# ambicuity/Distributed-LLM-Training-and-Inference-System

Hardware: AMD Instinct MI355X
Metric: tokens/sec (node) GPT-7B train (higher is better)
Workload: dtype bf16; 1 GPU; model=gpt-7b, global_batch=16, seq_len=2048, parallelism=dp1, micro_batch=16, grad_accum=1, activation_checkpoint=none, layout=planner

## Files before the change

llmctl/config/knobs.py:

```python

from __future__ import annotations

import contextlib
import dataclasses
import os
from dataclasses import dataclass, fields
from typing import Any, Dict, Iterator, Optional

ENV = "LLMCTL_KNOBS"


@dataclass(frozen=True)
class PerfKnobs:
    gemm64: bool = True
    gemm64_config: int = 304
    fwd64: str = "auto"
    dgrad64: str = "fused"
    wgrad_kernel: bool = True
    swiglu_bwd: str = "side"
    dgrad_transpose: bool = True
    wt_side_stream: bool = True
    fused_fwd: bool = False
    rope_inplace: bool = True
    fused_rope_attn: bool = True
    moe_pad: bool = True
    overlap_optimizer: bool = False
    gemm_tuning: bool = True
    fa_split: int = -1
    fa_prio: int = 1
    fa_nw: int = 4
    dkv: int = 2
    dkv_nwg: int = 0
    async_tp: bool = True
    async_tp_save_full: bool = False
    cp_zigzag: bool = True
    decode_fused: bool = True
    decode_splits: int = 0
    decode_v3: int = 1
    skinny_gemm: str = "auto"
    prefill_swiglu: bool = True
    prefill_fa: bool = True
    prefill_norm_fold: bool = True
    mixed_steps: bool = True
    custom_ar: bool = True
    tp_graphs: bool = True
    async_decode: bool = True
    tp_fused_decode: bool = True
    moe_decode_fused: bool = True

    def as_dict(self) -> Dict[str, Any]:
        return dataclasses.asdict(self)


NATIVE = ("fa_split", "fa_prio", "fa_nw", "dkv", "dkv_nwg", "decode_splits", "decode_v3")
_FIELDS = {f.name: f for f in fields(PerfKnobs)}


def _coerce(name: str, value: Any) -> Any:
    if name not in _FIELDS:
        raise KeyError(f"unknown performance knob {name!r} (known: {', '.join(sorted(_FIELDS))})")
    typ = _FIELDS[name].type
    if typ in ("bool", bool):
        if isinstance(value, str):
            v = value.strip().lower()
            if v not in ("1", "0", "true", "false", "on", "off", "yes", "no"):
                raise ValueError(f"knob {name}: expected a boolean, got {value!r}")
            return v in ("1", "true", "on", "yes")
        return bool(value)
    if typ in ("int", int):
        return int(value)
    return str(value)


def parse_env(spec: Optional[str]) -> Dict[str, Any]:
    out: Dict[str, Any] = {}
    for part in (spec or "").split(","):
        part = part.strip()
        if not part:
            continue
        if "=" not in part:
            raise ValueError(f"{ENV}: expected name=value, got {part!r}")
        k, v = part.split("=", 1)
        out[k.strip()] = _coerce(k.strip(), v.strip())
    return out


_RETIRED_ENV = ("LLMCTL_SIDE_DGRAD", "LLMCTL_DECODE_ATTN_QKV", "LLMCTL_GEMM64_CONFIG", "LLMCTL_SKINNY")
_warned: set = set()


def _warn_retired_env() -> None:
    import warnings

    names = [f"LLMCTL_{n.upper()}" for n in _FIELDS] + list(_RETIRED_ENV)
    for n in names:
        if n in os.environ and n not in _warned:
            _warned.add(n)
            warnings.warn(f"{n} is no longer read (performance switches are knobs now): set "
                          f"{ENV}=\"{n[7:].lower()}=<value>\" or the [perf] config table instead", stacklevel=3)


def resolve(overrides: Optional[Dict[str, Any]] = None, env: bool = True) -> PerfKnobs:
    _warn_retired_env()
    kw = {k: _coerce(k, v) for k, v in (overrides or {}).items()}
    if env:
        kw.update(parse_env(os.environ.get(ENV)))
    return PerfKnobs(**kw)


_ACTIVE: PerfKnobs = resolve()


def knobs() -> PerfKnobs:
    return _ACTIVE


def push_native(k: Optional[PerfKnobs] = None) -> bool:
    k = k or _ACTIVE
    try:
        from llmctl.ops import _lib

        if not _lib.loaded():
            return False
        import torch

        for name in NATIVE:
            torch.ops.llmctl.set_knob(name, int(getattr(k, name)))
        return True
    except Exception:
        return False


def apply(k: PerfKnobs) -> PerfKnobs:
    global _ACTIVE
    _ACTIVE = k
    push_native(k)
    return k


def use(k: PerfKnobs) -> PerfKnobs:
    if k is not _ACTIVE:
        apply(k)
    return k


def with_env(k: PerfKnobs) -> PerfKnobs:
    env = parse_env(os.environ.get(ENV))
    return dataclasses.replace(k, **env) if env else k


def configure(overrides: Optional[Dict[str, Any]] = None) -> PerfKnobs:
    return apply(resolve(overrides))


@contextlib.contextmanager
def override(**kw: Any) -> Iterator[PerfKnobs]:
    old = _ACTIVE
    new = dataclasses.replace(old, **{k: _coerce(k, v) for k, v in kw.items()})
    apply(new)
    try:
        yield new
    finally:
        apply(old)
```

llmctl/ops/csrc/flash_attn_fwd.hip:

```cpp
#include <cstdlib>

#include "attn_common.h"

namespace llmctl {
using namespace attn;
namespace {

constexpr int KB = 64;
constexpr float kRescaleTh = 8.f;

struct FwdArgs {
  const unsigned short* q;
  const unsigned short* k;
  const unsigned short* v;
  unsigned short* o;
  float* lse;
  int B, S, Hq, Hkv;
  long q_sb, q_ss, q_sh;
  long k_sb, k_ss, k_sh;
  long v_sb, v_ss, v_sh;
  long o_sb, o_ss, o_sh;
  float scale_log2;
  const int* doc;
  unsigned short* o_part;
  float* lse_part;
  int prio;
};

template <int HD, bool CAUSAL, bool DOC = false, bool SPLIT = false, int NW = 4, int NBUF = 2>
__global__ __launch_bounds__(NW * 64, 2) void fa_fwd_kernel(FwdArgs a) {
  constexpr int QB = NW * 32;
  constexpr int NTHR = NW * 64;
  constexpr int NKS = HD / 16;
  constexpr int NDB = HD / 32;
  constexpr int ROWB = HD * 2;
  constexpr int TILE = KB * ROWB;
  constexpr int PPW = TILE / 1024 / NW;
  constexpr int SLOT = 2 * TILE;
  static_assert(PPW * NW * 1024 == TILE, "pieces must split evenly over the waves");
  __shared__ __attribute__((aligned(1024))) unsigned char smem[NBUF * SLOT];

  const int tid = threadIdx.x;
  const int lane = tid & 63;
  const int wave = __builtin_amdgcn_readfirstlane(tid >> 6);
  const int r = lane & 31, hh = lane >> 5;
  const int nqb = (a.S + QB - 1) / QB;
  const int BH = a.B * a.Hq;
  int bh, rest;
  if (SPLIT || BH % 8) {
    bh = blockIdx.x % BH;
    rest = blockIdx.x / BH;
  } else {
    const int x = blockIdx.x & 7, j = blockIdx.x >> 3;
    bh = x * (BH >> 3) + j / nqb;
    rest = j % nqb;
  }
  const int part = SPLIT ? rest & 1 : 0;
  const int qblk = nqb - 1 - (SPLIT ? rest >> 1 : rest);
  const int b = bh / a.Hq, hq = bh % a.Hq;
  const int hk = hq / (a.Hq / a.Hkv);
  const int q_row0 = qblk * QB + wave * 32;
  const int my_q = q_row0 + r;

  const unsigned short* Qp = a.q + b * a.q_sb + hq * a.q_sh;
  const unsigned short* Kp = a.k + b * a.k_sb + hk * a.k_sh;
  const unsigned short* Vp = a.v + b * a.v_sb + hk * a.v_sh;

#pragma unroll
  for (int i = 0; i < NBUF * SLOT / (NTHR * 16); ++i)
    *reinterpret_cast<uint4*>(smem + i * NTHR * 16 + tid * 16) = make_uint4(0, 0, 0, 0);

  bf16x8_t qf[NKS];
#pragma unroll
  for (int ks = 0; ks < NKS; ++ks) {
    uint4 u = make_uint4(0, 0, 0, 0);
    if (my_q < a.S) u = gload16(Qp + (long)my_q * a.q_ss + ks * 16 + 8 * hh);
    qf[ks] = __builtin_bit_cast(bf16x8_t, u);
  }

  f32x16 o[NDB];
#pragma unroll
  for (int d = 0; d < NDB; ++d)
#pragma unroll
    for (int i = 0; i < 16; ++i) o[d][i] = 0.f;
  float m_i = -INFINITY, l_i = 0.f;

  const int kv_end = CAUSAL ? min(a.S, qblk * QB + QB) : a.S;
  int ntiles = (kv_end + KB - 1) / KB;
  int my_start = 0, w_min = 0, w_max = 0, t0 = 0;
  if constexpr (DOC) {
    const int* ds = a.doc + (long)b * a.S;
    my_start = ds[min(my_q, a.S - 1)];
    w_min = __builtin_amdgcn_readfirstlane(ds[min(q_row0, a.S - 1)]);
    w_max = __builtin_amdgcn_readfirstlane(ds[min(q_row0 + 31, a.S - 1)]);
    t0 = __builtin_amdgcn_readfirstlane(ds[min(qblk * QB, a.S - 1)]) / KB;
  }
  if constexpr (SPLIT) {
    const int mid = (t0 + ntiles) / 2;
    if (part == 0) ntiles = mid;
    else t0 = mid;
  }

  unsigned vk[PPW], vv[PPW];
#pragma unroll
  for (int i = 0; i < PPW; ++i) {
    const int byte = (i * NW + wave) * 1024 + lane * 16;
    const int row = byte / ROWB, pch = (byte % ROWB) >> 4;
    vk[i] = (unsigned)((row * a.k_ss + ((pch ^ swz_row<HD>(row)) << 3)) * 2);
    vv[i] = (unsigned)((row * a.v_ss + ((pch ^ swz_tr<HD>(row)) << 3)) * 2);
  }
  const unsigned lds0 = lds_addr(smem);
  int ik0 = t0 * KB;
  const unsigned short* kc = Kp + (long)ik0 * a.k_ss;
  const unsigned short* vc = Vp + (long)ik0 * a.v_ss;
  const long k_step = (long)KB * a.k_ss, v_step = (long)KB * a.v_ss;
  auto issue = [&](auto slot_c) __attribute__((always_inline)) {
    constexpr int SLC = decltype(slot_c)::value;
    const int nk = min(KB, a.S - ik0);
    i32x4_t rk = buf_rsrc(kc, (unsigned)(((nk - 1) * a.k_ss + HD) * 2));
    i32x4_t rv = buf_rsrc(vc, (unsigned)(((nk - 1) * a.v_ss + HD) * 2));
    asm volatile("s_nop 4" : "+s"(rk), "+s"(rv));
    const unsigned slot = lds0 + (unsigned)(SLC * SLOT) + wave * 1024;
#pragma unroll
    for (int i = 0; i < PPW; ++i) {
      buf_dma16(rk, vk[i], slot + i * NW * 1024);
      buf_dma16(rv, vv[i], slot + TILE + i * NW * 1024);
    }
    ik0 += KB;
    kc += k_step;
    vc += v_step;
  };

  const float c = a.scale_log2;
  const int key_hi = CAUSAL ? min(my_q, a.S - 1) : a.S - 1;
  int vlo[NDB], vhi[NDB];
#pragma unroll
  for (int d = 0; d < NDB; ++d) tr_frag_offs<HD>(d * 32, lane, vlo[d], vhi[d]);
  int kofs[NKS];
#pragma unroll
  for (int ks = 0; ks < NKS; ++ks) kofs[ks] = row_off<HD>(r, 2 * ks + hh);
#pragma unroll
  for (int ks = 0; ks < NKS; ++ks) asm volatile("" ::"v"(qf[ks]));
  auto tile = [&](bool need_mask, const unsigned char* Ks, const unsigned char* Vs, int kv0) __attribute__((always_inline)) {
    if (a.prio) __builtin_amdgcn_s_setprio(1);
    f32x16 s[2];
#pragma unroll
    for (int kb = 0; kb < 2; ++kb) {
#pragma unroll
      for (int i = 0; i < 16; ++i) s[kb][i] = 0.f;
#pragma unroll
      for (int ks = 0; ks < NKS; ++ks) s[kb] = mfma32(lds_read_b128(Ks, kb * 32 * (HD * 2) + kofs[ks]), qf[ks], s[kb]);
    }
    if (need_mask) {
#pragma unroll
      for (int kb = 0; kb < 2; ++kb)
#pragma unroll
        for (int i = 0; i < 16; ++i) {
          const int key = kv0 + kb * 32 + acc_row(i, hh);
          bool ok = key <= key_hi;
          if constexpr (DOC) ok = ok && key >= my_start;
          s[kb][i] = ok ? s[kb][i] : -INFINITY;
        }
    }
    if (a.prio) __builtin_amdgcn_s_setprio(0);
    float mx = s[0][0];
#pragma unroll
    for (int kb = 0; kb < 2; ++kb)
#pragma unroll
      for (int i = (kb == 0 ? 1 : 0); i < 16; ++i) mx = fmaxf(mx, s[kb][i]);
    mx = xor32_max(mx) * c;
    const bool grow = __builtin_amdgcn_ballot_w64(mx > m_i + kRescaleTh) != 0;
    const float m_new = grow ? fmaxf(m_i, mx) : m_i;
    const float nm = (m_new == -INFINITY) ? 0.f : -m_new;
    float rs = 0.f;
    bf16x8_t pb[2][2];
#pragma unroll
    for (int kb = 0; kb < 2; ++kb) {
      float p[16];
#pragma unroll
      for (int i = 0; i < 16; ++i) {
        p[i] = fast_exp2(__builtin_fmaf(s[kb][i], c, nm));
        rs += p[i];
      }
      pb[kb][0] = to_bf16x8(p);
      pb[kb][1] = to_bf16x8(p + 8);
    }
    rs = xor32_add(rs);
    if (grow) {
      const float alpha = fast_exp2(m_i + nm);
      l_i *= alpha;
#pragma unroll
      for (int d = 0; d < NDB; ++d)
#pragma unroll
        for (int i = 0; i < 16; ++i) o[d][i] *= alpha;
    }
    l_i += rs;
    m_i = m_new;
    if (a.prio) __builtin_amdgcn_s_setprio(1);
#pragma unroll
    for (int kb = 0; kb < 2; ++kb)
#pragma unroll
      for (int st = 0; st < 2; ++st)
#pragma unroll
        for (int d = 0; d < NDB; ++d) o[d] = mfma32(tr_frag_at<HD>(Vs, kb * 32 + 16 * st, vlo[d], vhi[d]), pb[kb][st], o[d]);
    if (a.prio) __builtin_amdgcn_s_setprio(0);
  };

  __syncthreads();
  auto step = [&](auto slot_c, int t) __attribute__((always_inline)) {
    constexpr int SL = decltype(slot_c)::value;
    if constexpr (NBUF == 3) {
      if (t + 1 < ntiles) vm_wait_n<2 * PPW>();
      else vm_wait_n<0>();
    } else {
      vm_wait_n<0>();
    }
    __builtin_amdgcn_s_barrier();
    if (t + NBUF - 1 < ntiles) issue(std::integral_constant<int, (SL + NBUF - 1) % NBUF>{});
    const int kv0 = t * KB;
    bool live = true;
    if constexpr (CAUSAL) live = kv0 <= q_row0 + 31;
    if constexpr (DOC) live = live && kv0 + KB > w_min;
    if (live) {
      const bool need_mask = (CAUSAL && kv0 + KB - 1 > q_row0) || (kv0 + KB > a.S) || (DOC && kv0 < w_max);
      tile(need_mask, smem + SL * SLOT, smem + SL * SLOT + TILE, kv0);
    }
  };
  if (t0 < ntiles) issue(std::integral_constant<int, 0>{});
  if constexpr (NBUF == 3)
    if (t0 + 1 < ntiles) issue(std::integral_constant<int, 1>{});
  for (int t = t0; t < ntiles; t += NBUF) {
    step(std::integral_constant<int, 0>{}, t);
    if (t + 1 < ntiles) step(std::integral_constant<int, 1>{}, t + 1);
    if constexpr (NBUF == 3)
      if (t + 2 < ntiles) step(std::integral_constant<int, 2>{}, t + 2);
  }

  if constexpr (SPLIT) {
    if (my_q < a.S) {
      const float inv = l_i > 0.f ? 1.f / l_i : 0.f;
      unsigned short* Op = a.o_part + ((((long)part * a.B + b) * a.S + my_q) * a.Hq + hq) * HD;
#pragma unroll
      for (int d = 0; d < NDB; ++d)
#pragma unroll
        for (int g = 0; g < 4; ++g) {
          const int col = d * 32 + 8 * g + 4 * hh;
          unsigned short w4[4];
#pragma unroll
          for (int j = 0; j < 4; ++j) w4[j] = f2bf(o[d][4 * g + j] * inv);
          *reinterpret_cast<uint2*>(Op + col) =
              make_uint2((unsigned)w4[0] | ((unsigned)w4[1] << 16), (unsigned)w4[2] | ((unsigned)w4[3] << 16));
        }
      if (hh == 0)
        a.lse_part[(((long)part * a.B + b) * a.Hq + hq) * a.S + my_q] =
            (l_i > 0.f) ? (m_i + __log2f(l_i)) * 0.69314718055994531f : -INFINITY;
    }
    return;
  }
  if (my_q < a.S) {
    const float inv = l_i > 0.f ? 1.f / l_i : 0.f;
    unsigned short* Op = a.o + b * a.o_sb + (long)my_q * a.o_ss + hq * a.o_sh;
#pragma unroll
    for (int d = 0; d < NDB; ++d)
#pragma unroll
      for (int g = 0; g < 4; ++g) {
        const int col = d * 32 + 8 * g + 4 * hh;
        unsigned short w4[4];
#pragma unroll
        for (int j = 0; j < 4; ++j) w4[j] = f2bf(o[d][4 * g + j] * inv);
        *reinterpret_cast<uint2*>(Op + col) =
            make_uint2((unsigned)w4[0] | ((unsigned)w4[1] << 16), (unsigned)w4[2] | ((unsigned)w4[3] << 16));
      }
    if (hh == 0) {
      const float lse = (l_i > 0.f) ? (m_i + __log2f(l_i)) * 0.69314718055994531f : -INFINITY;
      a.lse[((long)b * a.Hq + hq) * a.S + my_q] = lse;
    }
  }
}

template <int HD>
__global__ __launch_bounds__(256) void fa_combine_kernel(const unsigned short* __restrict__ o_part,
                                                         const float* __restrict__ lse_part,
                                                         unsigned short* __restrict__ o, float* __restrict__ lse,
                                                         int B, int S, int Hq, long o_sb, long o_ss, long o_sh) {
  constexpr int LPR = HD / 8;
  const long gid = (long)blockIdx.x * 256 + threadIdx.x;
  const long row = gid / LPR;
  const int sub = gid % LPR;
  if (row >= (long)B * S * Hq) return;
  const int hq = row % Hq;
  const long bs = row / Hq;
  const int sq = bs % S;
  const int b = bs / S;
  const long li = ((long)b * Hq + hq) * S + sq;
  const long plane = (long)B * Hq * S;
  const float l0 = lse_part[li], l1 = lse_part[plane + li];
  const float m = fmaxf(l0, l1);
  float w0 = 0.f, w1 = 0.f, l = -INFINITY;
  if (m != -INFINITY) {
    const float e0 = __expf(l0 - m), e1 = __expf(l1 - m);
    l = m + __logf(e0 + e1);
    w0 = e0 / (e0 + e1);
    w1 = e1 / (e0 + e1);
  }
  const long ob = row * HD + sub * 8;
  const long osz = (long)B * S * Hq * HD;
  float out[8], x0[8], x1[8];
  load8(o_part + ob, x0);
  load8(o_part + osz + ob, x1);
#pragma unroll
  for (int j = 0; j < 8; ++j) out[j] = w0 * x0[j] + w1 * x1[j];
  store8(o + b * o_sb + (long)sq * o_ss + (long)hq * o_sh + sub * 8, out);
  if (sub == 0) lse[li] = l;
}

template <int NW, int NBUF>
std::tuple<at::Tensor, at::Tensor> fwd_launch(const at::Tensor& q, at::Tensor& o, at::Tensor& lse, FwdArgs& a, int B,
                                              int S, int Hq, int D, bool causal,
                                              const c10::optional<at::Tensor>& doc_start) {
  constexpr int QB = NW * 32, WG_PER_CU = NW == 4 ? 2 : 1;
  const int nqb = (S + QB - 1) / QB;
  dim3 grid((unsigned)(B * Hq * nqb)), block(NW * 64);
  auto s = stream();
  bool split = causal && !(doc_start.has_value() && doc_start->defined()) && nqb >= 4 &&
               (long)B * Hq * nqb <= (long)WG_PER_CU * num_cus();
  if (const int64_t e = knob("fa_split", -1); e == 0) split = false;
  else if (e == 1) split = causal && !(doc_start.has_value() && doc_start->defined()) && nqb >= 2;
  if (split) {
    auto o_part = at::empty({2, B, S, Hq, D}, q.options());
    auto lse_part = at::empty({2, B, Hq, S}, q.options().dtype(at::kFloat));
    a.o_part = bf_mut(o_part);
    a.lse_part = lse_part.data_ptr<float>();
    dim3 g2((unsigned)(2 * B * Hq * nqb));
    const long threads = (long)B * S * Hq * (D / 8);
    if (D == 128) {
      hipLaunchKernelGGL((fa_fwd_kernel<128, true, false, true, NW, NBUF>), g2, block, 0, s, a);
      hipLaunchKernelGGL(fa_combine_kernel<128>, dim3((threads + 255) / 256), dim3(256), 0, s, a.o_part, a.lse_part,
                         bf_mut(o), lse.data_ptr<float>(), B, S, Hq, o.stride(0), o.stride(1), o.stride(2));
    } else {
      hipLaunchKernelGGL((fa_fwd_kernel<64, true, false, true, NW, NBUF>), g2, block, 0, s, a);
      hipLaunchKernelGGL(fa_combine_kernel<64>, dim3((threads + 255) / 256), dim3(256), 0, s, a.o_part, a.lse_part,
                         bf_mut(o), lse.data_ptr<float>(), B, S, Hq, o.stride(0), o.stride(1), o.stride(2));
    }
    return {o, lse};
  }
  if (doc_start.has_value() && doc_start->defined()) {
    const at::Tensor& ds = *doc_start;
    LLMCTL_CHECK(causal, "flash_attn_fwd: doc_start (packed sequences) needs causal attention");
    LLMCTL_CHECK(ds.is_cuda() && ds.scalar_type() == at::kInt && ds.is_contiguous() && ds.dim() == 2 &&
                     ds.size(0) == B && ds.size(1) == S,
                 "flash_attn_fwd: doc_start must be contiguous int32 [B,S]");
    a.doc = ds.data_ptr<int>();
    if (D == 128) hipLaunchKernelGGL((fa_fwd_kernel<128, true, true, false, NW, NBUF>), grid, block, 0, s, a);
    else hipLaunchKernelGGL((fa_fwd_kernel<64, true, true, false, NW, NBUF>), grid, block, 0, s, a);
    return {o, lse};
  }
  if (D == 128) {
    if (causal) hipLaunchKernelGGL((fa_fwd_kernel<128, true, false, false, NW, NBUF>), grid, block, 0, s, a);
    else hipLaunchKernelGGL((fa_fwd_kernel<128, false, false, false, NW, NBUF>), grid, block, 0, s, a);
  } else {
    if (causal) hipLaunchKernelGGL((fa_fwd_kernel<64, true, false, false, NW, NBUF>), grid, block, 0, s, a);
    else hipLaunchKernelGGL((fa_fwd_kernel<64, false, false, false, NW, NBUF>), grid, block, 0, s, a);
  }
  return {o, lse};
}

}

std::tuple<at::Tensor, at::Tensor> flash_attn_fwd(const at::Tensor& q, const at::Tensor& k, const at::Tensor& v,
                                                  double scale, bool causal,
                                                  const c10::optional<at::Tensor>& doc_start) {
  LLMCTL_CHECK(q.is_cuda() && k.is_cuda() && v.is_cuda(), "flash_attn_fwd: GPU tensors");
  LLMCTL_CHECK(q.scalar_type() == at::kBFloat16 && k.scalar_type() == at::kBFloat16 &&
                   v.scalar_type() == at::kBFloat16,
               "flash_attn_fwd: bf16");
  LLMCTL_CHECK(q.dim() == 4 && k.dim() == 4 && v.dim() == 4, "q/k/v must be [B,S,H,D]");
  const int B = q.size(0), S = q.size(1), Hq = q.size(2), D = q.size(3);
  const int Hkv = k.size(2);
  LLMCTL_CHECK(k.size(0) == B && k.size(1) == S && v.sizes() == k.sizes() && k.size(3) == D,
               "k/v shape must be [B,S,Hkv,D] matching q");
  LLMCTL_CHECK(Hq % Hkv == 0, "Hq must be a multiple of Hkv");
  LLMCTL_CHECK(D == 64 || D == 128, "head_dim must be 64 or 128, got ", D);
  LLMCTL_CHECK(q.stride(3) == 1 && k.stride(3) == 1 && v.stride(3) == 1, "head_dim must be contiguous");
  for (const at::Tensor* t : {&q, &k, &v})
    LLMCTL_CHECK(t->stride(0) % 8 == 0 && t->stride(1) % 8 == 0 && t->stride(2) % 8 == 0 &&
                     (reinterpret_cast<uintptr_t>(t->data_ptr()) & 15) == 0,
                 "q/k/v strides must be multiples of 8 elements and 16-B aligned");
  const c10::DeviceGuard g(q.device());
  auto o = at::empty({B, S, Hq, D}, q.options());
  auto lse = at::empty({B, Hq, S}, q.options().dtype(at::kFloat));
  if (B * S * Hq == 0) return {o, lse};
  FwdArgs a{bf_ptr(q), bf_ptr(k), bf_ptr(v), bf_mut(o), lse.data_ptr<float>(), B, S, Hq, Hkv,
            q.stride(0), q.stride(1), q.stride(2), k.stride(0), k.stride(1), k.stride(2),
            v.stride(0), v.stride(1), v.stride(2), o.stride(0), o.stride(1), o.stride(2),
            (float)(scale * 1.4426950408889634), nullptr, nullptr, nullptr, 0};
  a.prio = knob("fa_prio", 1) != 0 ? 1 : 0;
  if (knob("fa_nw", 4) == 8) return fwd_launch<8, 3>(q, o, lse, a, B, S, Hq, D, causal, doc_start);
  return fwd_launch<4, 2>(q, o, lse, a, B, S, Hq, D, causal, doc_start);
}

TORCH_LIBRARY_IMPL(llmctl, CUDA, m) { m.impl("flash_attn_fwd", &flash_attn_fwd); }

}
```

Before: 30910 tokens/s.

## Add paced two-head flash-attention forward kernel and MFMA/LDS-read schedule hints

Adds a new 512-thread forward attention kernel in which two 4-wave halves each handle one head. It uses a ring of LDS buffers and explicit barriers so that K/V DMA, softmax and the MFMA phases of consecutive tiles overlap in a paced pipeline. The kernel sits behind a new fa_paced knob that is off by default, and it includes optional timestamp instrumentation. Separately, sched_group_barrier hints that interleave LDS reads with MFMAs are inserted into the existing forward kernel, which changes instruction scheduling on the default path. The hints can help or hurt latency hiding, and the paced kernel gives up occupancy for tighter overlap.

```diff
diff --git a/llmctl/config/knobs.py b/llmctl/config/knobs.py
--- a/llmctl/config/knobs.py
+++ b/llmctl/config/knobs.py
@@ -29,6 +29,7 @@
     fa_split: int = -1
     fa_prio: int = 1
     fa_nw: int = 4
+    fa_paced: int = -1
     dkv: int = 2
     dkv_nwg: int = 0
     async_tp: bool = True
@@ -52,7 +53,7 @@
         return dataclasses.asdict(self)
 
 
-NATIVE = ("fa_split", "fa_prio", "fa_nw", "dkv", "dkv_nwg", "decode_splits", "decode_v3")
+NATIVE = ("fa_split", "fa_prio", "fa_nw", "fa_paced", "dkv", "dkv_nwg", "decode_splits", "decode_v3")
 _FIELDS = {f.name: f for f in fields(PerfKnobs)}
 
 
diff --git a/llmctl/ops/csrc/flash_attn_fwd.hip b/llmctl/ops/csrc/flash_attn_fwd.hip
--- a/llmctl/ops/csrc/flash_attn_fwd.hip
+++ b/llmctl/ops/csrc/flash_attn_fwd.hip
@@ -8,6 +8,8 @@
 
 constexpr int KB = 64;
 constexpr float kRescaleTh = 8.f;
+constexpr int kStampMax = 192;
+constexpr bool kPacedAuto = false;
 
 struct FwdArgs {
   const unsigned short* q;
@@ -27,6 +29,16 @@
   int prio;
 };
 
+template <int I, int N, int PF, int R>
+__device__ __forceinline__ void mfma_stream_sched() {
+  if constexpr (I == 0) __builtin_amdgcn_sched_group_barrier(0x100, R * PF, 0);
+  if constexpr (I < N) {
+    __builtin_amdgcn_sched_group_barrier(0x008, 1, 0);
+    if constexpr (I + PF < N) __builtin_amdgcn_sched_group_barrier(0x100, R, 0);
+    mfma_stream_sched<I + 1, N, PF, R>();
+  }
+}
+
 template <int HD, bool CAUSAL, bool DOC = false, bool SPLIT = false, int NW = 4, int NBUF = 2>
 __global__ __launch_bounds__(NW * 64, 2) void fa_fwd_kernel(FwdArgs a) {
   constexpr int QB = NW * 32;
@@ -151,6 +163,7 @@
 #pragma unroll
       for (int ks = 0; ks < NKS; ++ks) s[kb] = mfma32(lds_read_b128(Ks, kb * 32 * (HD * 2) + kofs[ks]), qf[ks], s[kb]);
     }
+    mfma_stream_sched<0, 2 * NKS, 4, 1>();
     if (need_mask) {
 #pragma unroll
       for (int kb = 0; kb < 2; ++kb)
@@ -203,6 +216,7 @@
       for (int st = 0; st < 2; ++st)
 #pragma unroll
         for (int d = 0; d < NDB; ++d) o[d] = mfma32(tr_frag_at<HD>(Vs, kb * 32 + 16 * st, vlo[d], vhi[d]), pb[kb][st], o[d]);
+    mfma_stream_sched<0, 4 * NDB, 4, 2>();
     if (a.prio) __builtin_amdgcn_s_setprio(0);
   };
 
@@ -257,6 +271,283 @@
     }
     return;
   }
+  if (my_q < a.S) {
+    const float inv = l_i > 0.f ? 1.f / l_i : 0.f;
+    unsigned short* Op = a.o + b * a.o_sb + (long)my_q * a.o_ss + hq * a.o_sh;
+#pragma unroll
+    for (int d = 0; d < NDB; ++d)
+#pragma unroll
+      for (int g = 0; g < 4; ++g) {
+        const int col = d * 32 + 8 * g + 4 * hh;
+        unsigned short w4[4];
+#pragma unroll
+        for (int j = 0; j < 4; ++j) w4[j] = f2bf(o[d][4 * g + j] * inv);
+        *reinterpret_cast<uint2*>(Op + col) =
+            make_uint2((unsigned)w4[0] | ((unsigned)w4[1] << 16), (unsigned)w4[2] | ((unsigned)w4[3] << 16));
+      }
+    if (hh == 0) {
+      const float lse = (l_i > 0.f) ? (m_i + __log2f(l_i)) * 0.69314718055994531f : -INFINITY;
+      a.lse[((long)b * a.Hq + hq) * a.S + my_q] = lse;
+    }
+  }
+}
+
+__device__ __forceinline__ void seg_barrier() {
+  __builtin_amdgcn_sched_barrier(0);
+  __builtin_amdgcn_s_barrier();
+  __builtin_amdgcn_sched_barrier(0);
+}
+
+template <int HD, bool CAUSAL>
+__global__ __launch_bounds__(512, 1) void fa_fwd_paced_kernel(FwdArgs a) {
+  constexpr int NW = 4;
+  constexpr int QB = NW * 32;
+  constexpr int NKS = HD / 16;
+  constexpr int NDB = HD / 32;
+  constexpr int ROWB = HD * 2;
+  constexpr int TILE = KB * ROWB;
+  constexpr int PPW = TILE / 1024 / NW;
+  constexpr int SLOT = 2 * TILE;
+  constexpr int RING = 2 * SLOT;
+  __shared__ __attribute__((aligned(1024))) unsigned char smem[2 * RING];
+
+  const int tid = threadIdx.x;
+  const int lane = tid & 63;
+#ifdef LLMCTL_FA_STAMP
+  __shared__ unsigned long long stamp_lds[8 * kStampMax];
+  int nst = 0;
+  const bool stamping = a.lse_part != nullptr && blockIdx.x == gridDim.x / 2;
+  auto stamp = [&]() __attribute__((always_inline)) {
+    if (stamping && nst < kStampMax) {
+      const unsigned long long now = __builtin_amdgcn_s_memrealtime();
+      if (lane == 0) stamp_lds[(tid >> 6) * kStampMax + nst] = now;
+      ++nst;
+    }
+  };
+#else
+  auto stamp = [&]() __attribute__((always_inline)) {};
+#endif
+  const int half = __builtin_amdgcn_readfirstlane(tid >> 8);
+  const int wave = __builtin_amdgcn_readfirstlane((tid >> 6) & 3);
+  const int r = lane & 31, hh = lane >> 5;
+  const int nqb = (a.S + QB - 1) / QB;
+  const int NP = (a.B * a.Hq) >> 1;
+  int pair, rest;
+  if (NP % 8) {
+    pair = blockIdx.x % NP;
+    rest = blockIdx.x / NP;
+  } else {
+    const int x = blockIdx.x & 7, j = blockIdx.x >> 3;
+    pair = x * (NP >> 3) + j / nqb;
+    rest = j % nqb;
+  }
+  const int bh = 2 * pair + half;
+  const int qblk = nqb - 1 - rest;
+  const int b = bh / a.Hq, hq = bh % a.Hq;
+  const int hk = hq / (a.Hq / a.Hkv);
+  const int q_row0 = qblk * QB + wave * 32;
+  const int my_q = q_row0 + r;
+
+  const unsigned short* Qp = a.q + b * a.q_sb + hq * a.q_sh;
+  const unsigned short* Kp = a.k + b * a.k_sb + hk * a.k_sh;
+  const unsigned short* Vp = a.v + b * a.v_sb + hk * a.v_sh;
+
+#pragma unroll
+  for (int i = 0; i < 2 * RING / (512 * 16); ++i)
+    *reinterpret_cast<uint4*>(smem + i * 512 * 16 + tid * 16) = make_uint4(0, 0, 0, 0);
+
+  bf16x8_t qf[NKS];
+#pragma unroll
+  for (int ks = 0; ks < NKS; ++ks) {
+    uint4 u = make_uint4(0, 0, 0, 0);
+    if (my_q < a.S) u = gload16(Qp + (long)my_q * a.q_ss + ks * 16 + 8 * hh);
+    qf[ks] = __builtin_bit_cast(bf16x8_t, u);
+  }
+
+  f32x16 o[NDB];
+#pragma unroll
+  for (int d = 0; d < NDB; ++d)
+#pragma unroll
+    for (int i = 0; i < 16; ++i) o[d][i] = 0.f;
+  float m_i = -INFINITY, l_i = 0.f;
+
+  const int kv_end = CAUSAL ? min(a.S, qblk * QB + QB) : a.S;
+  const int ntiles = (kv_end + KB - 1) / KB;
+
+  unsigned vk[PPW], vv[PPW];
+#pragma unroll
+  for (int i = 0; i < PPW; ++i) {
+    const int byte = (i * NW + wave) * 1024 + lane * 16;
+    const int row = byte / ROWB, pch = (byte % ROWB) >> 4;
+    vk[i] = (unsigned)((row * a.k_ss + ((pch ^ swz_row<HD>(row)) << 3)) * 2);
+    vv[i] = (unsigned)((row * a.v_ss + ((pch ^ swz_tr<HD>(row)) << 3)) * 2);
+  }
+  const unsigned lds0 = lds_addr(smem) + (unsigned)(half * RING);
+  int ikk = 0, ikv = 0;
+  const unsigned short* kc = Kp;
+  const unsigned short* vc = Vp;
+  const long k_step = (long)KB * a.k_ss, v_step = (long)KB * a.v_ss;
+  auto issue_k = [&](auto slot_c) __attribute__((always_inline)) {
+    constexpr int SLC = decltype(slot_c)::value;
+    const int nk = min(KB, a.S - ikk);
+    i32x4_t rk = buf_rsrc(kc, (unsigned)(((nk - 1) * a.k_ss + HD) * 2));
+    asm volatile("s_nop 4" : "+s"(rk));
+    const unsigned slot = lds0 + (unsigned)(SLC * SLOT) + wave * 1024;
+#pragma unroll
+    for (int i = 0; i < PPW; ++i) buf_dma16(rk, vk[i], slot + i * NW * 1024);
+    ikk += KB;
+    kc += k_step;
+  };
+  auto issue_v = [&](auto slot_c) __attribute__((always_inline)) {
+    constexpr int SLC = decltype(slot_c)::value;
+    const int nk = min(KB, a.S - ikv);
+    i32x4_t rv = buf_rsrc(vc, (unsigned)(((nk - 1) * a.v_ss + HD) * 2));
+    asm volatile("s_nop 4" : "+s"(rv));
+    const unsigned slot = lds0 + (unsigned)(SLC * SLOT + TILE) + wave * 1024;
+#pragma unroll
+    for (int i = 0; i < PPW; ++i) buf_dma16(rv, vv[i], slot + i * NW * 1024);
+    ikv += KB;
+    vc += v_step;
+  };
+
+  const float c = a.scale_log2;
+  const int key_hi = CAUSAL ? min(my_q, a.S - 1) : a.S - 1;
+  int vlo[NDB], vhi[NDB];
+#pragma unroll
+  for (int d = 0; d < NDB; ++d) {
+    tr_frag_offs<HD>(d * 32, lane, vlo[d], vhi[d]);
+    vlo[d] += half * RING;
+    vhi[d] += half * RING;
+  }
+  int kofs[NKS];
+#pragma unroll
+  for (int ks = 0; ks < NKS; ++ks) kofs[ks] = row_off<HD>(r, 2 * ks + hh) + half * RING;
+#pragma unroll
+  for (int ks = 0; ks < NKS; ++ks) asm volatile("" ::"v"(qf[ks]));
+
+  f32x16 s[2];
+  bf16x8_t pb[2][2];
+  auto is_live = [&](int t) __attribute__((always_inline)) {
+    return !CAUSAL || t * KB <= q_row0 + 31;
+  };
+  auto m1 = [&](auto slot_c, int t) __attribute__((always_inline)) {
+    constexpr int SL = decltype(slot_c)::value;
+    if (!is_live(t)) return;
+    const unsigned char* Ks = smem + SL * SLOT;
+    const int kv0 = t * KB;
+#pragma unroll
+    for (int kb = 0; kb < 2; ++kb) {
+#pragma unroll
+      for (int i = 0; i < 16; ++i) s[kb][i] = 0.f;
+#pragma unroll
+      for (int ks = 0; ks < NKS; ++ks) s[kb] = mfma32(lds_read_b128(Ks, kb * 32 * (HD * 2) + kofs[ks]), qf[ks], s[kb]);
+    }
+    mfma_stream_sched<0, 2 * NKS, 4, 1>();
+    const bool need_mask = (CAUSAL && kv0 + KB - 1 > q_row0) || (kv0 + KB > a.S);
+    if (need_mask) {
+#pragma unroll
+      for (int kb = 0; kb < 2; ++kb)
+#pragma unroll
+        for (int i = 0; i < 16; ++i) {
+          const int key = kv0 + kb * 32 + acc_row(i, hh);
+          s[kb][i] = key <= key_hi ? s[kb][i] : -INFINITY;
+        }
+    }
+  };
+  auto xs = [&](int t) __attribute__((always_inline)) {
+    if (!is_live(t)) return;
+    float mx = s[0][0];
+#pragma unroll
+    for (int kb = 0; kb < 2; ++kb)
+#pragma unroll
+      for (int i = (kb == 0 ? 1 : 0); i < 16; ++i) mx = fmaxf(mx, s[kb][i]);
+    mx = xor32_max(mx) * c;
+    const bool grow = __builtin_amdgcn_ballot_w64(mx > m_i + kRescaleTh) != 0;
+    const float m_new = grow ? fmaxf(m_i, mx) : m_i;
+    const float nm = (m_new == -INFINITY) ? 0.f : -m_new;
+    float rs = 0.f;
+#pragma unroll
+    for (int kb = 0; kb < 2; ++kb) {
+      float p[16];
+#pragma unroll
+      for (int i = 0; i < 16; ++i) {
+        p[i] = fast_exp2(__builtin_fmaf(s[kb][i], c, nm));
+        rs += p[i];
+      }
+      pb[kb][0] = to_bf16x8(p);
+      pb[kb][1] = to_bf16x8(p + 8);
+    }
+    rs = xor32_add(rs);
+    if (grow) {
+      const float alpha = fast_exp2(m_i + nm);
+      l_i *= alpha;
+#pragma unroll
+      for (int d = 0; d < NDB; ++d)
+#pragma unroll
+        for (int i = 0; i < 16; ++i) o[d][i] *= alpha;
+    }
+    l_i += rs;
+    m_i = m_new;
+  };
+  auto m2 = [&](auto slot_c, int t) __attribute__((always_inline)) {
+    constexpr int SL = decltype(slot_c)::value;
+    if (!is_live(t)) return;
+    const unsigned char* Vs = smem + SL * SLOT + TILE;
+#pragma unroll
+    for (int kb = 0; kb < 2; ++kb)
+#pragma unroll
+      for (int st = 0; st < 2; ++st)
+#pragma unroll
+        for (int d = 0; d < NDB; ++d) o[d] = mfma32(tr_frag_at<HD>(Vs, kb * 32 + 16 * st, vlo[d], vhi[d]), pb[kb][st], o[d]);
+    mfma_stream_sched<0, 4 * NDB, 4, 2>();
+  };
+  auto step = [&](auto slot_c, int t) __attribute__((always_inline)) {
+    constexpr int SL = decltype(slot_c)::value;
+    seg_barrier();
+    stamp();
+    if (t + 2 < ntiles) issue_k(slot_c);
+    if (t + 1 < ntiles) issue_v(std::integral_constant<int, SL ^ 1>{});
+    xs(t);
+    stamp();
+    if (t + 2 < ntiles) vm_wait_n<2 * PPW>();
+    else if (t + 1 < ntiles) vm_wait_n<PPW>();
+    else vm_wait_n<0>();
+    stamp();
+    seg_barrier();
+    stamp();
+    if (a.prio) __builtin_amdgcn_s_setprio(1);
+    m2(slot_c, t);
+    if (t + 1 < ntiles) m1(std::integral_constant<int, SL ^ 1>{}, t + 1);
+    if (a.prio) __builtin_amdgcn_s_setprio(0);
+    stamp();
+  };
+
+  __syncthreads();
+  issue_k(std::integral_constant<int, 0>{});
+  issue_v(std::integral_constant<int, 0>{});
+  if (ntiles > 1) issue_k(std::integral_constant<int, 1>{});
+  if (half) seg_barrier();
+  if (ntiles > 1) vm_wait_n<2 * PPW>();
+  else vm_wait_n<PPW>();
+  seg_barrier();
+  if (a.prio) __builtin_amdgcn_s_setprio(1);
+  m1(std::integral_constant<int, 0>{}, 0);
+  if (a.prio) __builtin_amdgcn_s_setprio(0);
+  for (int t = 0; t < ntiles; t += 2) {
+    step(std::integral_constant<int, 0>{}, t);
+    if (t + 1 < ntiles) step(std::integral_constant<int, 1>{}, t + 1);
+  }
+  if (!half) seg_barrier();
+#ifdef LLMCTL_FA_STAMP
+  if (stamping && lane == 0) {
+    unsigned long long* out = reinterpret_cast<unsigned long long*>(a.lse_part);
+    const int w8 = tid >> 6;
+    for (int i = 0; i < nst; ++i) out[w8 * kStampMax + i] = stamp_lds[w8 * kStampMax + i];
+    out[8 * kStampMax + w8] = (unsigned long long)nst;
+    return;
+  }
+#endif
+
   if (my_q < a.S) {
     const float inv = l_i > 0.f ? 1.f / l_i : 0.f;
     unsigned short* Op = a.o + b * a.o_sb + (long)my_q * a.o_ss + hq * a.o_sh;
@@ -354,6 +645,18 @@
     if (D == 128) hipLaunchKernelGGL((fa_fwd_kernel<128, true, true, false, NW, NBUF>), grid, block, 0, s, a);
     else hipLaunchKernelGGL((fa_fwd_kernel<64, true, true, false, NW, NBUF>), grid, block, 0, s, a);
     return {o, lse};
+  }
+  if constexpr (NW == 4) {
+    const int64_t paced = knob("fa_paced", -1);
+    if (D == 128 && (B * Hq) % 2 == 0 && (paced == 1 || (paced < 0 && kPacedAuto))) {
+      dim3 gp((unsigned)(B * Hq / 2 * nqb));
+#ifdef LLMCTL_FA_STAMP
+      if (lse.numel() * 4 >= (long)(8 * kStampMax + 8) * 8) a.lse_part = lse.data_ptr<float>();
+#endif
+      if (causal) hipLaunchKernelGGL((fa_fwd_paced_kernel<128, true>), gp, dim3(512), 0, s, a);
+      else hipLaunchKernelGGL((fa_fwd_paced_kernel<128, false>), gp, dim3(512), 0, s, a);
+      return {o, lse};
+    }
   }
   if (D == 128) {
     if (causal) hipLaunchKernelGGL((fa_fwd_kernel<128, true, false, false, NW, NBUF>), grid, block, 0, s, a);
```

New measurement: 30910 tokens/s. No clear change (-0.0%).
